# caojiezhang/CiaoSR

Hardware: AMD Instinct MI355X
Metric: HR Mpix/s (RDN-CiaoSR x4, LocalImplicitSR forward_test) (higher is better)
Workload: dtype f32; 1 GPU; C3: RDN-CiaoSR (c64b16) x4, LR 1356x2040 -> 5424x8160 (DIV2K-shaped 2K LR), tiled inference: 117 tiles of 192x192 (overlap 32), random-init weights, fp32; scale=4, tiles=117, parallelism=tile-shard x1

## Files before the change

ciaosr_amd/csrc/csa_attn_v4_f32.hip:

```cpp
#include "ops.h"

namespace ciaosr {

typedef float f32x16 __attribute__((ext_vector_type(16)));
typedef int i32x4 __attribute__((ext_vector_type(4)));

constexpr int AV_KW = 10;
constexpr int AV_SW = 2 * AV_KW;
constexpr int AV_RS = AV_SW + 3;
constexpr int AV_C = 64;
constexpr int AV_NCOL = 4 * AV_KW;
constexpr int AV_BT = AV_NCOL * AV_C;
constexpr int AV_KP = AV_NCOL / 2;
constexpr int AV_SA = 14;
constexpr int AV_SB = 8;
constexpr int AV_PF = 4;
static_assert(AV_SA % 2 == 0 && AV_SB % 2 == 0 && AV_PF % 2 == 0 && AV_KP % 2 == 0 && AV_SA > 0 && AV_SA + AV_PF <= AV_KP && AV_SB > 0 &&
              AV_SB < AV_KP, "k-pair groups; half 1 is not read before the barrier that completes it");

template <int QW>
struct AvCfg {
    static constexpr int NP = 256;
    static constexpr int NT = 2 * NP + 64 * (QW / 48);
    static constexpr int TR = NP / AV_RS;
    static constexpr int NI = (QW + 3 + TR - 1) / TR;
    static constexpr int NRB = TR * NI;
    static constexpr int PST = 4 * NRB * AV_RS;
    static constexpr int AT = AV_NCOL * QW;
    static constexpr size_t LDS = (size_t)(2 * AV_BT + PST + 2 * AT) * sizeof(float);
};
static_assert(AvCfg<192>::LDS <= 163840 && AvCfg<96>::LDS <= 163840, "LDS");
static_assert(AvCfg<192>::NP >= 192 + AV_KW - 1 && AvCfg<96>::NP >= 96 + AV_KW - 1, "one thread per diagonal");
static_assert(AvCfg<192>::NRB >= 192 + 3 && AvCfg<96>::NRB >= 96 + 3, "staged rows");
static_assert(2 * AV_BT >= (AV_KW - 1) * AV_RS && 2 * AvCfg<96>::AT >= (AV_KW + 2) * AV_RS + AV_RS, "diagonal read guard");

#ifdef CIAOSR_PROBE
__device__ unsigned long long g_avprobe[1024 * 48];
#define AVPROBE_T() __builtin_readcyclecounter()
#else
#define AVPROBE_T() 0ull
#endif

struct CsaAv4P {
    const float* S; const float2* st; const float* Pc; float* part;
    int Hp, Wp, Hh, Wh, Lld, nseg, nch, n_wg;
    int ys, oy0, noy;
    unsigned s_bytes, pc_bytes;
};

__device__ __forceinline__ void av_phase_barrier() {
    asm volatile("" ::: "memory");
    __builtin_amdgcn_s_barrier();
    asm volatile("" ::: "memory");
}

template <int QW>
__global__ __launch_bounds__(AvCfg<QW>::NT) void csa_attn_v4_kernel(CsaAv4P p) {
    using Cfg = AvCfg<QW>;
    constexpr int NP = Cfg::NP, TR = Cfg::TR, NI = Cfg::NI, NRB = Cfg::NRB;
    constexpr int NB = (AV_BT / 4 + NP - 1) / NP;
    extern __shared__ __attribute__((aligned(16))) float avs[];
    float* Bt = avs;
    float* Pst = avs + 2 * AV_BT;
    float* At = Pst + Cfg::PST;

    const int bid = blockIdx.x;
    const int q8 = p.n_wg >> 3, r8 = p.n_wg & 7;
    const int xcd = bid & 7, slot0 = bid >> 3;
    const int lid = (xcd < r8 ? xcd * (q8 + 1) : r8 * (q8 + 1) + (xcd - r8) * q8) + slot0;
    const int oy = p.oy0 + lid % p.noy, rest = lid / p.noy;
    const int seg = rest % p.nseg, quarter = rest / p.nseg;
    const int x0 = seg * QW, nq = min(QW, p.Wp - x0);
    const int ngy = p.Hh + 3, gyb = quarter * ngy / 4, nr = (quarter + 1) * ngy / 4 - gyb;
    const int HWp = p.Hp * p.Wp;
    const int nsteps = nr * p.nch;

    const int t = threadIdx.x, lane = t & 63, w = __builtin_amdgcn_readfirstlane(t >> 6);
#ifdef CIAOSR_PROBE
    const bool stamp = QW == 192 && lane == 0 && (w & 3) == 0 && bid < 1024;
    unsigned long long pacc[10] = {0, 0, 0, 0, 0, 0, 0, 0, 0, 0};
    const unsigned long long pstart = AVPROBE_T();
#define AVPROBE_ADD(slot, t0) do { const unsigned long long now_ = AVPROBE_T(); pacc[slot] += now_ - (t0); (t0) = now_; } while (0)
#define AVPROBE_OUT(role) do { if (stamp) { for (int i_ = 0; i_ < 10; ++i_) g_avprobe[bid * 48 + 16 * (role) + i_] = pacc[i_];                \
        g_avprobe[bid * 48 + 16 * (role) + 14] = AVPROBE_T() - pstart; g_avprobe[bid * 48 + 16 * (role) + 15] = (unsigned long long)nsteps; } } while (0)
#else
#define AVPROBE_ADD(slot, t0) do { } while (0)
#define AVPROBE_OUT(role) do { } while (0)
#endif

    int trow = 0, ch = 0;
    int gy = gyb + oy % nr, gx0 = 0;
    auto next_step = [&]() __attribute__((always_inline)) {
        if (++ch == p.nch) { ch = 0; ++trow; }
        gy = gyb + (trow + oy) % nr; gx0 = ch * AV_SW;
    };

    if (w < NP / 64) {
        const __amdgpu_buffer_rsrc_t rs_s = __builtin_amdgcn_make_buffer_rsrc(const_cast<float*>(p.S), 0, p.s_bytes, 0x00020000);
        const bool stager = t < TR * AV_RS;
        const int sj = t % AV_RS, sr0 = t / AV_RS;
        float negm[4][NI];
#pragma unroll
        for (int dyi = 0; dyi < 4; ++dyi) {
            const int qy = oy + dyi - 2;
#pragma unroll
            for (int i = 0; i < NI; ++i) {
                const int qx = x0 + sr0 + TR * i - 2;
                float v = -__builtin_inff();
                if (stager && qy >= 0 && qy < p.Hp && qx >= 0 && qx < p.Wp) {
                    const float2 s2 = p.st[(size_t)qy * p.Wp + qx];
                    v = -(s2.x - __builtin_amdgcn_logf(s2.y));
                }
                negm[dyi][i] = v;
            }
        }
        const int s_thread = sr0 * p.Lld + sj;
        const int s_istep = TR * p.Lld;
        float ra[4][NI];
        auto issue_logits = [&](auto dy0_c) __attribute__((always_inline)) {
            constexpr int DY0 = decltype(dy0_c)::value;
#pragma unroll
            for (int dyi = DY0; dyi < DY0 + 2; ++dyi) {
                const int dy = dyi - 2;
                const int base = ((oy + dy - p.ys) * p.Wp + x0 - 2) * p.Lld + (gy - 1 + dy) * p.Wh + gx0 - 3 + s_thread;
#pragma unroll
                for (int i = 0; i < NI; ++i)
                    ra[dyi][i] = __int_as_float(__builtin_amdgcn_raw_buffer_load_b32(rs_s, (base + i * s_istep) * 4, 0, 0));
            }
        };
        auto stage = [&](auto edge_c) __attribute__((always_inline)) {
            constexpr bool EDGE = decltype(edge_c)::value;
            constexpr float kL2e = 1.4426950408889634f;
            const bool kx = (unsigned)(gx0 - 3 + sj) < (unsigned)p.Wh;
#pragma unroll
            for (int dyi = 0; dyi < 4; ++dyi) {
                const bool ok = kx && (unsigned)(gy - 3 + dyi) < (unsigned)p.Hh;
                float* dst = Pst + dyi * NRB * AV_RS + sr0 * AV_RS + sj;
#pragma unroll
                for (int i = 0; i < NI; ++i) {
                    float v = __builtin_amdgcn_exp2f(__builtin_fmaf(ra[dyi][i], kL2e, negm[dyi][i]));
                    if (EDGE) v = ok ? v : 0.f;
                    if (stager) dst[i * TR * AV_RS] = v;
                }
                __builtin_amdgcn_sched_barrier(0);
            }
        };
        issue_logits(std::integral_constant<int, 0>{});
        issue_logits(std::integral_constant<int, 2>{});
        [[maybe_unused]] unsigned long long pt0 = AVPROBE_T();
#pragma unroll 1
        for (int step = 0; step < nsteps; ++step) {
            const bool edge = gy < 3 || gy >= p.Hh || gx0 < 3 || gx0 + AV_SW - 1 >= p.Wh;
            if (edge) stage(std::true_type{});
            else stage(std::false_type{});
            AVPROBE_ADD(0, pt0);
            __syncthreads();
            AVPROBE_ADD(1, pt0);
            next_step();
            const bool more = step + 1 < nsteps;
            if (more) issue_logits(std::integral_constant<int, 0>{});
            AVPROBE_ADD(2, pt0);
            __syncthreads();
            AVPROBE_ADD(3, pt0);
            if (more) issue_logits(std::integral_constant<int, 2>{});
            AVPROBE_ADD(4, pt0);
            __syncthreads();
            AVPROBE_ADD(5, pt0);
        }
        AVPROBE_OUT(0);
        return;
    }

    if (w < 2 * NP / 64) {
        const int td = t - NP;
        const __amdgpu_buffer_rsrc_t rs_pc = __builtin_amdgcn_make_buffer_rsrc(const_cast<float*>(p.Pc), 0, p.pc_bytes, 0x00020000);
        int b_rel[NB], b_k[NB];
#pragma unroll
        for (int s = 0; s < NB; ++s) {
            const int idx = td + NP * s, kk = idx >> 4, c4 = idx & 15;
            const int blk = kk / AV_KW, k = kk - blk * AV_KW;
            const int pcb = blk == 0 ? 8 : blk == 1 ? 6 : blk == 2 ? 2 : 0;
            b_rel[s] = k * 9 * AV_C + pcb * AV_C + 4 * c4;
            b_k[s] = idx < AV_BT / 4 ? k : 0x40000000;
        }
        float4 rb[2][NB];
        auto issue_u = [&]() __attribute__((always_inline)) {
#pragma unroll
            for (int h = 0; h < 2; ++h) {
                const int brow = (gy * (p.Wh + 3) + gx0 + AV_KW * h) * 9 * AV_C;
#pragma unroll
                for (int s = 0; s < NB; ++s) {
                    const unsigned off = gx0 + AV_KW * h + b_k[s] < p.Wh + 3 ? (unsigned)(brow + b_rel[s]) * 4u : 0x80000000u;
                    const i32x4 v = __builtin_amdgcn_raw_buffer_load_b128(rs_pc, off, 0, 0);
                    rb[h][s] = make_float4(__int_as_float(v.x), __int_as_float(v.y), __int_as_float(v.z), __int_as_float(v.w));
                }
            }
        };
        const int c = td - (AV_KW - 1);
        const bool diag = td < QW + AV_KW - 1;
        const float* dsrc = Pst + c * AV_RS;
        float* adst0 = At + c;
        auto half = [&](auto h_c) __attribute__((always_inline)) {
            constexpr int H = decltype(h_c)::value;
#pragma unroll
            for (int s = 0; s < NB; ++s)
                if (NP * (s + 1) <= AV_BT / 4 || td + NP * s < AV_BT / 4)
                    *reinterpret_cast<float4*>(Bt + H * AV_BT + 4 * (td + NP * s)) = rb[H][s];
            if (diag) {
                float* adst = adst0 + H * Cfg::AT;
                float xa2[AV_KW], xb2[AV_KW], ya[AV_KW], yb[AV_KW];
#pragma unroll
                for (int dyi = 0; dyi < 4; ++dyi) {
                    float d[AV_KW + 3];
#pragma unroll
                    for (int j = 0; j < AV_KW + 3; ++j) d[j] = dsrc[dyi * NRB * AV_RS + AV_KW * H + j * (AV_RS + 1)];
#pragma unroll
                    for (int k = 0; k < AV_KW; ++k) {
                        const float pr = d[k + 1] + d[k + 2];
                        const float xa = pr + d[k + 3], xb = pr + d[k];
                        if (dyi == 0) { xa2[k] = xa; xb2[k] = xb; }
                        else if (dyi == 1) { ya[k] = xa; yb[k] = xb; }
                        else if (dyi == 2) {
                            ya[k] = ya[k] + xa; yb[k] = yb[k] + xb;
                            if ((unsigned)(c + k) < (unsigned)nq) {
                                adst[(2 * AV_KW + k) * QW + k] = ya[k] + xa2[k];
                                adst[(3 * AV_KW + k) * QW + k] = yb[k] + xb2[k];
                            }
                        } else if ((unsigned)(c + k) < (unsigned)nq) {
                            adst[(0 * AV_KW + k) * QW + k] = ya[k] + xa;
                            adst[(1 * AV_KW + k) * QW + k] = yb[k] + xb;
                        }
                    }
                }
            }
        };
        [[maybe_unused]] unsigned long long pt0 = AVPROBE_T();
#pragma unroll 1
        for (int step = 0; step < nsteps; ++step) {
            issue_u();
            __syncthreads();
            AVPROBE_ADD(0, pt0);
            half(std::integral_constant<int, 0>{});
            AVPROBE_ADD(1, pt0);
            __syncthreads();
            AVPROBE_ADD(2, pt0);
            half(std::integral_constant<int, 1>{});
            next_step();
            AVPROBE_ADD(3, pt0);
            __syncthreads();
            AVPROBE_ADD(4, pt0);
        }
        AVPROBE_OUT(1);
        return;
    }

    const int cw = w - 2 * NP / 64, wm = cw >> 1, wn = cw & 1, li = lane & 31, lh = lane >> 5;
    f32x16 acc[3];
#pragma unroll
    for (int mi = 0; mi < 3; ++mi)
#pragma unroll
        for (int r = 0; r < 16; ++r) acc[mi][r] = 0.f;
    const float* fa = At + lh * QW + wm * 96 + li;
    const float* fb = Bt + lh * AV_C + wn * 32 + li;
    [[maybe_unused]] unsigned long long ct0 = AVPROBE_T();
    auto mma_step = [&](auto nbar_c) __attribute__((always_inline)) {
        constexpr int NBAR = decltype(nbar_c)::value, NE = 2 * AV_KP;
        float a[NE][3], b[NE];
        auto ld = [&](int e) __attribute__((always_inline)) {
            const int h = e / AV_KP, kp = e - h * AV_KP;
            b[e] = fb[h * AV_BT + 2 * kp * AV_C];
#pragma unroll
            for (int mi = 0; mi < 3; ++mi) a[e][mi] = fa[h * Cfg::AT + 2 * kp * QW + mi * 32];
        };
#pragma unroll
        for (int e = 0; e < AV_PF; ++e) ld(e);
#pragma unroll
        for (int e = 0; e < NE; e += 2) {
            if (e + AV_PF < NE) { ld(e + AV_PF); ld(e + AV_PF + 1); }
            __builtin_amdgcn_sched_barrier(0);
#pragma unroll
            for (int u = 0; u < 2; ++u)
#pragma unroll
                for (int mi = 0; mi < 3; ++mi)
                    acc[mi] = __builtin_amdgcn_mfma_f32_32x32x2f32(a[e + u][mi], b[e + u], acc[mi], 0, 0, 0);
            __builtin_amdgcn_sched_barrier(0);
            if (NBAR >= 1 && e + 2 == AV_SA) {
                AVPROBE_ADD(0, ct0);
                av_phase_barrier();
                AVPROBE_ADD(1, ct0);
            }
            if (NBAR >= 2 && e + 2 == AV_KP + AV_SB) {
                AVPROBE_ADD(2, ct0);
                av_phase_barrier();
                AVPROBE_ADD(3, ct0);
            }
        }
    };
    if (nsteps > 0) {
        av_phase_barrier();
        __syncthreads();
    }
    ct0 = AVPROBE_T();
#pragma unroll 1
    for (int step = 0; step + 1 < nsteps; ++step) {
        mma_step(std::integral_constant<int, 2>{});
        AVPROBE_ADD(4, ct0);
        __syncthreads();
        AVPROBE_ADD(5, ct0);
    }
    if (nsteps > 0) mma_step(std::integral_constant<int, 1>{});
    AVPROBE_OUT(2);

    float* dst = p.part + ((size_t)quarter * HWp + (size_t)oy * p.Wp + x0) * AV_C + wn * 32 + li;
#pragma unroll
    for (int mi = 0; mi < 3; ++mi)
#pragma unroll
        for (int r = 0; r < 16; ++r) {
            const int row = wm * 96 + mi * 32 + (r & 3) + 8 * (r >> 2) + 4 * lh;
            if (row < nq) dst[(size_t)row * AV_C] = acc[mi][r];
        }
}
#undef AVPROBE_ADD
#undef AVPROBE_OUT


__device__ __forceinline__ int av_subset(int d) { return d == -2 ? 0 : (d == 1 ? 2 : 1); }

__global__ void csa_gather_vedge_kernel(const float* __restrict__ Pc, int Hh, int Wh, int C, float* __restrict__ Ve) {
    const int c4n = C >> 2;
    const long n = (long)Hh * Wh * 9 * c4n;
    const int We = Wh + 3;
    for (long idx = blockIdx.x * (long)blockDim.x + threadIdx.x; idx < n; idx += (long)gridDim.x * blockDim.x) {
        const int c4 = (int)(idx % c4n);
        const long t = idx / c4n;
        const int blk = (int)(t % 9);
        const int l = (int)(t / 9);
        const int ly = l / Wh, lx = l - ly * Wh;
        int dy, dx, r, sct;
        if (blk < 4) { dy = 0; dx = blk - 2; r = 0; sct = av_subset(dx); }
        else if (blk < 8) { dy = blk - 6; dx = 0; r = av_subset(dy); sct = 0; }
        else { dy = 0; dx = 0; r = 0; sct = 0; }
        const size_t src = ((size_t)(ly - dy + 1) * We + (lx - dx + 1)) * (9 * C) + (size_t)(3 * r + sct) * C + 4 * c4;
        reinterpret_cast<float4*>(Ve)[idx] = *reinterpret_cast<const float4*>(Pc + src);
    }
}

__global__ void csa_attn_v4_combine_kernel(const float* __restrict__ part, const float* __restrict__ Otop, const float* __restrict__ Oleft,
                                           const float* __restrict__ Otl, const float* __restrict__ bd, int H, int W, int Hp, int Wp,
                                           int C, float* __restrict__ out, int ld_out) {
    const int c4n = C >> 2;
    const long n = (long)H * W * c4n;
    const size_t qs = (size_t)Hp * Wp * C;
    for (long idx = blockIdx.x * (long)blockDim.x + threadIdx.x; idx < n; idx += (long)gridDim.x * blockDim.x) {
        const int c4 = (int)(idx % c4n);
        const long pix = idx / c4n;
        const int x = (int)(pix % W), y = (int)(pix / W);
        const size_t o = ((size_t)y * Wp + x) * C + 4 * c4;
        float4 acc = *reinterpret_cast<const float4*>(part + o);
#pragma unroll
        for (int q = 1; q < 4; ++q) {
            const float4 v = *reinterpret_cast<const float4*>(part + q * qs + o);
            acc.x += v.x; acc.y += v.y; acc.z += v.z; acc.w += v.w;
        }
        if (y == 0 || x == 0) {
            float4 e = make_float4(0.f, 0.f, 0.f, 0.f);
            if (y == 0)
                for (int dx = -2; dx <= 1; ++dx) {
                    if (x + dx < 0 || x + dx >= Wp) continue;
                    const float4 v = *reinterpret_cast<const float4*>(Otop + (size_t)(x + dx) * 4 * C + (size_t)(dx + 2) * C + 4 * c4);
                    e.x += v.x; e.y += v.y; e.z += v.z; e.w += v.w;
                }
            if (x == 0)
                for (int dy = -2; dy <= 1; ++dy) {
                    if (y + dy < 0 || y + dy >= Hp) continue;
                    const float4 v = *reinterpret_cast<const float4*>(Oleft + (size_t)(y + dy) * 4 * C + (size_t)(dy + 2) * C + 4 * c4);
                    e.x += v.x; e.y += v.y; e.z += v.z; e.w += v.w;
                }
            if (y == 0 && x == 0) {
                const float4 v = *reinterpret_cast<const float4*>(Otl + 4 * c4);
                e.x -= v.x; e.y -= v.y; e.z -= v.z; e.w -= v.w;
            }
            acc.x -= e.x; acc.y -= e.y; acc.z -= e.z; acc.w -= e.w;
        }
        const float4 b = *reinterpret_cast<const float4*>(bd + 4 * c4);
        acc.x = (b.x + acc.x) / 6.f; acc.y = (b.y + acc.y) / 6.f; acc.z = (b.z + acc.z) / 6.f; acc.w = (b.w + acc.w) / 6.f;
        *reinterpret_cast<float4*>(out + (size_t)pix * ld_out + 4 * c4) = acc;
    }
}

static inline int av_grid(long n) {
    long g = (n + 255) / 256;
    return (int)(g < 1 ? 1 : (g > 4096 ? 4096 : g));
}

bool csa_attn_v4_ok(int Hp, int Wp, int C, int Lld, int s_rows) {
    return C == AV_C && Hp >= 4 && Wp >= 4 && (Hp & 1) == 0 && (Wp & 1) == 0 && (Lld & 3) == 0 && s_rows >= 1 &&
           (size_t)s_rows * Wp * Lld * sizeof(float) < 0x80000000ull;
}

int csa_attn_v4_f32(const float* S, int Lld, const float* stats2, const float* Pc, float* part, int Hp, int Wp, int C, bool tile128,
                    int ys, int s_rows, int oy0, int oy1, hipStream_t s) {
    CIAOSR_CHECK_ARG(S && stats2 && Pc && part && csa_attn_v4_ok(Hp, Wp, C, Lld, s_rows) && aligned16(Pc) && aligned16(part));
    CIAOSR_CHECK_ARG(0 <= oy0 && oy0 < oy1 && oy1 <= Hp && ys >= 0 && ys + s_rows <= Hp && ys <= (oy0 > 2 ? oy0 - 2 : 0) &&
                     ys + s_rows >= (oy1 < Hp ? oy1 + 1 : Hp));
    CsaAv4P p;
    p.S = S; p.st = reinterpret_cast<const float2*>(stats2); p.Pc = Pc; p.part = part;
    p.Hp = Hp; p.Wp = Wp; p.Hh = Hp / 2; p.Wh = Wp / 2; p.Lld = Lld;
    const int qw = tile128 ? 96 : 192;
    p.nseg = ceil_div(Wp, qw);
    p.nch = ceil_div(p.Wh + 3, AV_SW);
    p.ys = ys; p.oy0 = oy0; p.noy = oy1 - oy0;
    p.n_wg = p.noy * p.nseg * 4;
    p.s_bytes = (unsigned)((size_t)s_rows * Wp * Lld * sizeof(float));
    p.pc_bytes = (unsigned)((size_t)(p.Hh + 3) * (p.Wh + 3) * 9 * C * sizeof(float));
    ProfScope prof("csa_attn_v", s);
    if (tile128) {
        CIAOSR_BIG_LDS(csa_attn_v4_kernel<96>, AvCfg<96>::LDS);
        hipLaunchKernelGGL(csa_attn_v4_kernel<96>, dim3(p.n_wg), dim3(AvCfg<96>::NT), AvCfg<96>::LDS, s, p);
    } else {
        CIAOSR_BIG_LDS(csa_attn_v4_kernel<192>, AvCfg<192>::LDS);
        hipLaunchKernelGGL(csa_attn_v4_kernel<192>, dim3(p.n_wg), dim3(AvCfg<192>::NT), AvCfg<192>::LDS, s, p);
    }
    return launch_status("csa_attn_v4_f32");
}

int csa_gather_vedge(const float* Pc, int Hh, int Wh, int C, float* Ve, hipStream_t s) {
    ProfScope prof("csa_gather_vedge", s);
    hipLaunchKernelGGL(csa_gather_vedge_kernel, dim3(av_grid((long)Hh * Wh * 9 * C / 4)), dim3(256), 0, s, Pc, Hh, Wh, C, Ve);
    return launch_status("csa_gather_vedge");
}

int csa_attn_v4_combine(const float* part, const float* Otop, const float* Oleft, const float* Otl, const float* bd, int H, int W, int Hp,
                        int Wp, int C, float* out, int ld_out, hipStream_t s) {
    ProfScope prof("csa_gather_out", s);
    hipLaunchKernelGGL(csa_attn_v4_combine_kernel, dim3(av_grid((long)H * W * C / 4)), dim3(256), 0, s, part, Otop, Oleft, Otl, bd, H, W,
                       Hp, Wp, C, out, ld_out);
    return launch_status("csa_attn_v4_combine");
}

}

#ifdef CIAOSR_PROBE
extern "C" int ciaosr_debug_probe_av4_read(unsigned long long* host, int n_words) {
    return hipMemcpyFromSymbol(host, HIP_SYMBOL(ciaosr::g_avprobe), (size_t)n_words * 8) == hipSuccess ? 0 : -1;
}
#endif
```

ciaosr_amd/csrc/csa_scores_f32.hip:

```cpp
#include "ops.h"

namespace ciaosr {

typedef float f32x16 __attribute__((ext_vector_type(16)));
typedef int i32x4 __attribute__((ext_vector_type(4)));

constexpr int BSH = 8, BSW = 16;
constexpr int BLH = 4, BLW = 16;
constexpr int BHW = BSW + 2;
constexpr int BPN = (BSH + 2) * BHW;
constexpr int BLN = (BLH + 2) * BHW;
constexpr int BDP = 109;
constexpr int BDB = BPN * BDP * 4;
constexpr size_t kBoxLds = 2 * (size_t)BDB;
constexpr unsigned kOobB = 0xFFFFFFF0u;

struct BoxP {
    const float* M; int ldm; unsigned m_bytes; int Hp, Wp;
    int y0, y1;
    const float* R; int ldr; unsigned r_bytes; int Hl, Wl;
    const float* nrm;
    float* S; int lds_; size_t s_floats;
    int pbx, lbx, n_lb, n_items;
};

__global__ void csa_key_norms_kernel(const float* __restrict__ R, int ldr, int Hl, int Wl, int Ch, float floor_, float alpha,
                                     float* __restrict__ nrm) {
    const int lane = threadIdx.x & 63;
    const long l = (long)blockIdx.x * 4 + (threadIdx.x >> 6);
    if (l >= (long)Hl * Wl) return;
    const int ly = (int)(l / Wl), lx = (int)(l - (long)ly * Wl);
    float ss = 0.f;
    for (int e = lane; e < 9 * Ch; e += 64) {
        const int tap = e / Ch, c = e - tap * Ch;
        const int y = ly + tap / 3 - 1, x = lx + tap % 3 - 1;
        if (y >= 0 && y < Hl && x >= 0 && x < Wl) {
            const float v = R[((size_t)y * Wl + x) * ldr + c];
            ss += v * v;
        }
    }
#pragma unroll
    for (int o = 32; o > 0; o >>= 1) ss += __shfl_xor(ss, o, 64);
    if (lane == 0) nrm[l] = alpha / fmaxf(sqrtf(ss), floor_);
}

__global__ __launch_bounds__(512) void csa_scores_box_f32_kernel(BoxP p) {
    extern __shared__ __attribute__((aligned(16))) float Dl[];
    const int t = threadIdx.x, lane = t & 63, wv = __builtin_amdgcn_readfirstlane(t >> 6), li = lane & 31, lh = lane >> 5;
    const int per = (p.n_items + (int)gridDim.x - 1) / (int)gridDim.x;
    const int i0 = (int)blockIdx.x * per, i1 = min(i0 + per, p.n_items);
    if (i0 >= i1) return;
    auto item_pb = [&](int it) -> int { return it / p.n_lb; };
    auto item_lb = [&](int it) -> int { return it - (it / p.n_lb) * p.n_lb; };

    if (wv < 4) {
        const __amdgpu_buffer_rsrc_t rs_m = __builtin_amdgcn_make_buffer_rsrc(const_cast<float*>(p.M), 0, p.m_bytes, 0x00020000);
        const __amdgpu_buffer_rsrc_t rs_r = __builtin_amdgcn_make_buffer_rsrc(const_cast<float*>(p.R), 0, p.r_bytes, 0x00020000);
        auto row_off = [&](int h, int hn, int y0, int x0, int Hh, int Ww, int ld) -> unsigned {
            const int hy = h / BHW, hx = h - hy * BHW;
            const int y = y0 - 1 + hy, x = x0 - 1 + hx;
            return (h < hn && y >= 0 && y < Hh && x >= 0 && x < Ww) ? (unsigned)(((size_t)y * Ww + x) * ld * 4) + (unsigned)lh * 16u : kOobB;
        };
        i32x4 fa[6][4];
        i32x4 fbc[4], fbn[4];
        auto load_a = [&](int pb) {
            const int py0 = p.y0 + (pb / p.pbx) * BSH, px0 = (pb % p.pbx) * BSW;
#pragma unroll
            for (int pt = 0; pt < 6; ++pt) {
                const unsigned mo = row_off(32 * pt + li, BPN, py0, px0, p.Hp, p.Wp, p.ldm);
#pragma unroll
                for (int j = 0; j < 4; ++j) fa[pt][j] = __builtin_amdgcn_raw_buffer_load_b128(rs_m, mo == kOobB ? (int)kOobB : (int)(mo + 32u * j), 0, 0);
            }
        };
        auto load_b = [&](int lb, i32x4 (&f)[4]) {
            const int ly0 = (lb / p.lbx) * BLH, lx0 = (lb % p.lbx) * BLW;
            const unsigned ro = row_off(32 * wv + li, BLN, ly0, lx0, p.Hl, p.Wl, p.ldr);
#pragma unroll
            for (int j = 0; j < 4; ++j) f[j] = __builtin_amdgcn_raw_buffer_load_b128(rs_r, ro == kOobB ? (int)kOobB : (int)(ro + 32u * j), 0, 0);
        };
        int cur_pb = item_pb(i0);
        load_a(cur_pb);
        load_b(item_lb(i0), fbc);
#pragma unroll 1
        for (int it = i0; it <= i1; ++it) {
            if (it < i1) {
                const int k = (it - i0) & 1;
                if (it + 1 < i1) load_b(item_lb(it + 1), fbn);
                float* D = Dl + k * (BDB / 4);
                const int lcol = 32 * wv + li;
#pragma unroll
                for (int pt = 0; pt < 6; ++pt) {
                    f32x16 acc;
#pragma unroll
                    for (int e = 0; e < 16; ++e) acc[e] = 0.f;
#pragma unroll
                    for (int j = 0; j < 4; ++j) {
                        const i32x4 a = fa[pt][j], b = fbc[j];
                        acc = __builtin_amdgcn_mfma_f32_32x32x2f32(__int_as_float(a.x), __int_as_float(b.x), acc, 0, 0, 0);
                        acc = __builtin_amdgcn_mfma_f32_32x32x2f32(__int_as_float(a.y), __int_as_float(b.y), acc, 0, 0, 0);
                        acc = __builtin_amdgcn_mfma_f32_32x32x2f32(__int_as_float(a.z), __int_as_float(b.z), acc, 0, 0, 0);
                        acc = __builtin_amdgcn_mfma_f32_32x32x2f32(__int_as_float(a.w), __int_as_float(b.w), acc, 0, 0, 0);
                    }
                    if (lcol < BLN) {
                        float* dcol = D + (4 * lh) * BDP + lcol;
#pragma unroll
                        for (int r = 0; r < 16; ++r) {
                            constexpr int kLast = BPN - 1;
                            const int rr = 32 * pt + (r & 3) + 8 * (r >> 2);
                            if (rr + 4 <= kLast) dcol[rr * BDP] = acc[r];
                            else if (rr <= kLast && lh == 0) dcol[rr * BDP] = acc[r];
                        }
                    }
                }
#pragma unroll
                for (int j = 0; j < 4; ++j) fbc[j] = fbn[j];
                if (it + 1 < i1 && item_pb(it + 1) != cur_pb) {
                    cur_pb = item_pb(it + 1);
                    load_a(cur_pb);
                }
            }
            __syncthreads();
        }
    } else {
        const int lyy = lane >> 4, lxx = lane & 15;
        int lcol9[9];
#pragma unroll
        for (int a = 0; a < 3; ++a)
#pragma unroll
            for (int b = 0; b < 3; ++b) lcol9[3 * a + b] = (lyy + a) * BHW + lxx + b;
        const int q0 = 32 * (wv - 4);
#pragma unroll 1
        for (int it = i0; it <= i1; ++it) {
            if (it > i0) {
                const int ci = it - 1, k = (ci - i0) & 1;
                const int pb = item_pb(ci), lb = item_lb(ci);
                const int py0 = p.y0 + (pb / p.pbx) * BSH, px0 = (pb % p.pbx) * BSW;
                const int ly = (lb / p.lbx) * BLH + lyy, lx = (lb % p.lbx) * BLW + lxx;
                const bool l_ok = ly < p.Hl && lx < p.Wl;
                const float sc = l_ok ? p.nrm[(size_t)ly * p.Wl + lx] : 0.f;
                const float* D = Dl + k * (BDB / 4) + (q0 >> 4) * BHW * BDP;
                const unsigned lane_off = l_ok ? (unsigned)((size_t)ly * p.Wl + lx) * 4u : kOobB;
                const int qy0 = py0 + (q0 >> 4);
                const size_t s_base = ((size_t)(qy0 - p.y0) * p.Wp + px0) * p.lds_;
                const size_t s_left = p.s_floats > s_base ? (p.s_floats - s_base) * 4 : 0;
                const size_t s_span = ((size_t)p.Wp + BSW) * p.lds_ * 4;
                const __amdgpu_buffer_rsrc_t rs_s =
                    __builtin_amdgcn_make_buffer_rsrc(p.S + s_base, 0, (unsigned)(s_left < s_span ? s_left : s_span), 0x00020000);
                const float* dk[9];
#pragma unroll
                for (int e = 0; e < 9; ++e) dk[e] = D + lcol9[e];
#pragma unroll
                for (int q = 0; q < 32; ++q) {
                    const int pyy = q >> 4, pxx = q & 15;
                    float s = dk[0][(pyy * BHW + pxx) * BDP];
#pragma unroll
                    for (int e = 1; e < 9; ++e) s += dk[e][((pyy + e / 3) * BHW + pxx + e % 3) * BDP];
                    const bool row_ok = qy0 + pyy < p.y1 && px0 + pxx < p.Wp;
                    const unsigned soff = (unsigned)(((size_t)pyy * p.Wp + pxx) * p.lds_ * 4);
                    __builtin_amdgcn_raw_buffer_store_b32(__float_as_int(s * sc), rs_s, (int)(row_ok ? lane_off : kOobB), (int)(row_ok ? soff : 0u), 0);
                }
            }
            __syncthreads();
        }
    }
}

bool csa_scores_box_ok(int Ch, int ldm, int ldr) { return Ch == 32 && (ldm & 3) == 0 && (ldr & 3) == 0; }

int csa_key_norms(const float* R, int ldr, int Hl, int Wl, int Ch, float alpha, float floor_, float* nrm, hipStream_t s) {
    CIAOSR_CHECK_ARG(R && nrm && csa_scores_box_ok(Ch, Ch, ldr));
    ProfScope prof("csa_key_norms", s);
    hipLaunchKernelGGL(csa_key_norms_kernel, dim3(ceil_div((long)Hl * Wl, 4)), dim3(256), 0, s, R, ldr, Hl, Wl, Ch, floor_, alpha, nrm);
    return launch_status("csa_key_norms");
}

int csa_scores_box_f32(const float* M, int ldm, int Hp, int Wp, const float* R, int ldr, int Hl, int Wl, int Ch, const float* nrm, float* S,
                       int ld_s, int y0, int y1, hipStream_t s) {
    CIAOSR_CHECK_ARG(M && R && nrm && S && csa_scores_box_ok(Ch, ldm, ldr) && aligned16(M) && aligned16(R) && 0 <= y0 && y0 < y1 && y1 <= Hp);
    const size_t mb = (size_t)Hp * Wp * ldm * 4, rb = (size_t)Hl * Wl * ldr * 4;
    const size_t s_floats = ((size_t)(y1 - y0) * Wp - 1) * ld_s + (size_t)Hl * Wl;
    CIAOSR_CHECK_ARG(mb < 0xFFFFFF00ull && rb < 0xFFFFFF00ull && ((size_t)Wp + BSW) * ld_s * 4 < 0xFFFFFF00ull);
    BoxP p;
    p.M = M; p.ldm = ldm; p.m_bytes = (unsigned)mb; p.Hp = Hp; p.Wp = Wp; p.y0 = y0; p.y1 = y1;
    p.R = R; p.ldr = ldr; p.r_bytes = (unsigned)rb; p.Hl = Hl; p.Wl = Wl;
    p.nrm = nrm; p.S = S; p.lds_ = ld_s; p.s_floats = s_floats;
    p.pbx = ceil_div(Wp, BSW); p.lbx = ceil_div(Wl, BLW);
    p.n_lb = ceil_div(Hl, BLH) * p.lbx;
    const long n_items = (long)ceil_div(y1 - y0, BSH) * p.pbx * p.n_lb;
    CIAOSR_CHECK_ARG(n_items < 0x7FFFFFFF);
    p.n_items = (int)n_items;
    CIAOSR_BIG_LDS(csa_scores_box_f32_kernel, kBoxLds);
    ProfScope prof("csa_scores", s);
    hipLaunchKernelGGL(csa_scores_box_f32_kernel, dim3(p.n_items < 256 ? p.n_items : 256), dim3(512), kBoxLds, s, p);
    return launch_status("csa_scores_box_f32");
}

}
```

Before: 12.15 Mpix/s.

## Pack attention and score-box LDS math into paired f32x2 ops with aligned blocks

Measured after the change: 12.21 Mpix/s (median of 6 runs). No clear change (+0.5%).

```diff
diff --git a/ciaosr_amd/csrc/csa_attn_v4_f32.hip b/ciaosr_amd/csrc/csa_attn_v4_f32.hip
--- a/ciaosr_amd/csrc/csa_attn_v4_f32.hip
+++ b/ciaosr_amd/csrc/csa_attn_v4_f32.hip
@@ -4,6 +4,8 @@
 
 typedef float f32x16 __attribute__((ext_vector_type(16)));
 typedef int i32x4 __attribute__((ext_vector_type(4)));
+typedef float f32x2 __attribute__((ext_vector_type(2)));
+typedef __attribute__((address_space(3))) const float* av_lds_cptr;
 
 constexpr int AV_KW = 10;
 constexpr int AV_SW = 2 * AV_KW;
@@ -25,13 +27,15 @@
     static constexpr int TR = NP / AV_RS;
     static constexpr int NI = (QW + 3 + TR - 1) / TR;
     static constexpr int NRB = TR * NI;
-    static constexpr int PST = 4 * NRB * AV_RS;
+    static constexpr int PB = (NRB * AV_RS + 63) / 64 * 64;
+    static constexpr int PST = 4 * PB;
     static constexpr int AT = AV_NCOL * QW;
     static constexpr size_t LDS = (size_t)(2 * AV_BT + PST + 2 * AT) * sizeof(float);
 };
 static_assert(AvCfg<192>::LDS <= 163840 && AvCfg<96>::LDS <= 163840, "LDS");
 static_assert(AvCfg<192>::NP >= 192 + AV_KW - 1 && AvCfg<96>::NP >= 96 + AV_KW - 1, "one thread per diagonal");
 static_assert(AvCfg<192>::NRB >= 192 + 3 && AvCfg<96>::NRB >= 96 + 3, "staged rows");
+static_assert(3 * AvCfg<192>::PB / 64 < 256 && AvCfg<192>::PB % 64 == 0 && AvCfg<96>::PB % 64 == 0, "ds_read2st64_b32 offsets of the four blocks");
 static_assert(2 * AV_BT >= (AV_KW - 1) * AV_RS && 2 * AvCfg<96>::AT >= (AV_KW + 2) * AV_RS + AV_RS, "diagonal read guard");
 
 #ifdef CIAOSR_PROBE
@@ -57,7 +61,7 @@
 template <int QW>
 __global__ __launch_bounds__(AvCfg<QW>::NT) void csa_attn_v4_kernel(CsaAv4P p) {
     using Cfg = AvCfg<QW>;
-    constexpr int NP = Cfg::NP, TR = Cfg::TR, NI = Cfg::NI, NRB = Cfg::NRB;
+    constexpr int NP = Cfg::NP, TR = Cfg::TR, NI = Cfg::NI, PB = Cfg::PB;
     constexpr int NB = (AV_BT / 4 + NP - 1) / NP;
     extern __shared__ __attribute__((aligned(16))) float avs[];
     float* Bt = avs;
@@ -99,7 +103,7 @@
         const __amdgpu_buffer_rsrc_t rs_s = __builtin_amdgcn_make_buffer_rsrc(const_cast<float*>(p.S), 0, p.s_bytes, 0x00020000);
         const bool stager = t < TR * AV_RS;
         const int sj = t % AV_RS, sr0 = t / AV_RS;
-        float negm[4][NI];
+        f32x2 negm[4][(NI + 1) / 2];
 #pragma unroll
         for (int dyi = 0; dyi < 4; ++dyi) {
             const int qy = oy + dyi - 2;
@@ -111,7 +115,7 @@
                     const float2 s2 = p.st[(size_t)qy * p.Wp + qx];
                     v = -(s2.x - __builtin_amdgcn_logf(s2.y));
                 }
-                negm[dyi][i] = v;
+                negm[dyi][i >> 1][i & 1] = v;
             }
         }
         const int s_thread = sr0 * p.Lld + sj;
@@ -135,12 +139,18 @@
 #pragma unroll
             for (int dyi = 0; dyi < 4; ++dyi) {
                 const bool ok = kx && (unsigned)(gy - 3 + dyi) < (unsigned)p.Hh;
-                float* dst = Pst + dyi * NRB * AV_RS + sr0 * AV_RS + sj;
-#pragma unroll
-                for (int i = 0; i < NI; ++i) {
-                    float v = __builtin_amdgcn_exp2f(__builtin_fmaf(ra[dyi][i], kL2e, negm[dyi][i]));
-                    if (EDGE) v = ok ? v : 0.f;
-                    if (stager) dst[i * TR * AV_RS] = v;
+                float* dst = Pst + dyi * PB + sr0 * AV_RS + sj;
+#pragma unroll
+                for (int i = 0; i < NI; i += 2) {
+                    f32x2 e;
+                    if (i + 1 < NI) e = __builtin_elementwise_fma(f32x2{ra[dyi][i], ra[dyi][i + 1]}, f32x2{kL2e, kL2e}, negm[dyi][i >> 1]);
+                    else e.x = __builtin_fmaf(ra[dyi][i], kL2e, negm[dyi][i >> 1].x);
+#pragma unroll
+                    for (int u = 0; u < 2 && i + u < NI; ++u) {
+                        float v = __builtin_amdgcn_exp2f(e[u]);
+                        if (EDGE) v = ok ? v : 0.f;
+                        if (stager) dst[(i + u) * TR * AV_RS] = v;
+                    }
                 }
                 __builtin_amdgcn_sched_barrier(0);
             }
@@ -198,7 +208,14 @@
         };
         const int c = td - (AV_KW - 1);
         const bool diag = td < QW + AV_KW - 1;
-        const float* dsrc = Pst + c * AV_RS;
+        av_lds_cptr dsrc[2][AV_KW + 3];
+#pragma unroll
+        for (int h = 0; h < 2; ++h)
+#pragma unroll
+            for (int j = 0; j < AV_KW + 3; ++j) {
+                dsrc[h][j] = (av_lds_cptr)(Pst + c * AV_RS + AV_KW * h + j * (AV_RS + 1));
+                asm volatile("" : "+v"(dsrc[h][j]));
+            }
         float* adst0 = At + c;
         auto half = [&](auto h_c) __attribute__((always_inline)) {
             constexpr int H = decltype(h_c)::value;
@@ -208,27 +225,25 @@
                     *reinterpret_cast<float4*>(Bt + H * AV_BT + 4 * (td + NP * s)) = rb[H][s];
             if (diag) {
                 float* adst = adst0 + H * Cfg::AT;
-                float xa2[AV_KW], xb2[AV_KW], ya[AV_KW], yb[AV_KW];
-#pragma unroll
-                for (int dyi = 0; dyi < 4; ++dyi) {
-                    float d[AV_KW + 3];
-#pragma unroll
-                    for (int j = 0; j < AV_KW + 3; ++j) d[j] = dsrc[dyi * NRB * AV_RS + AV_KW * H + j * (AV_RS + 1)];
+                f32x2 xa01[AV_KW], xb01[AV_KW];
+#pragma unroll
+                for (int pr_i = 0; pr_i < 2; ++pr_i) {
+                    f32x2 d[AV_KW + 3];
+#pragma unroll
+                    for (int j = 0; j < AV_KW + 3; ++j) d[j] = f32x2{dsrc[H][j][2 * pr_i * PB], dsrc[H][j][(2 * pr_i + 1) * PB]};
 #pragma unroll
                     for (int k = 0; k < AV_KW; ++k) {
-                        const float pr = d[k + 1] + d[k + 2];
-                        const float xa = pr + d[k + 3], xb = pr + d[k];
-                        if (dyi == 0) { xa2[k] = xa; xb2[k] = xb; }
-                        else if (dyi == 1) { ya[k] = xa; yb[k] = xb; }
-                        else if (dyi == 2) {
-                            ya[k] = ya[k] + xa; yb[k] = yb[k] + xb;
+                        const f32x2 pr = d[k + 1] + d[k + 2];
+                        const f32x2 xa = pr + d[k + 3], xb = pr + d[k];
+                        if (pr_i == 0) { xa01[k] = xa; xb01[k] = xb; }
+                        else {
+                            const float ya = xa01[k].y + xa.x, yb = xb01[k].y + xb.x;
                             if ((unsigned)(c + k) < (unsigned)nq) {
-                                adst[(2 * AV_KW + k) * QW + k] = ya[k] + xa2[k];
-                                adst[(3 * AV_KW + k) * QW + k] = yb[k] + xb2[k];
+                                adst[(2 * AV_KW + k) * QW + k] = ya + xa01[k].x;
+                                adst[(3 * AV_KW + k) * QW + k] = yb + xb01[k].x;
+                                adst[(0 * AV_KW + k) * QW + k] = ya + xa.y;
+                                adst[(1 * AV_KW + k) * QW + k] = yb + xb.y;
                             }
-                        } else if ((unsigned)(c + k) < (unsigned)nq) {
-                            adst[(0 * AV_KW + k) * QW + k] = ya[k] + xa;
-                            adst[(1 * AV_KW + k) * QW + k] = yb[k] + xb;
                         }
                     }
                 }
diff --git a/ciaosr_amd/csrc/csa_scores_f32.hip b/ciaosr_amd/csrc/csa_scores_f32.hip
--- a/ciaosr_amd/csrc/csa_scores_f32.hip
+++ b/ciaosr_amd/csrc/csa_scores_f32.hip
@@ -4,6 +4,7 @@
 
 typedef float f32x16 __attribute__((ext_vector_type(16)));
 typedef int i32x4 __attribute__((ext_vector_type(4)));
+typedef float f32x2 __attribute__((ext_vector_type(2)));
 
 constexpr int BSH = 8, BSW = 16;
 constexpr int BLH = 4, BLW = 16;
@@ -14,6 +15,13 @@
 constexpr int BDB = BPN * BDP * 4;
 constexpr size_t kBoxLds = 2 * (size_t)BDB;
 constexpr unsigned kOobB = 0xFFFFFFF0u;
+
+#ifdef CIAOSR_PROBE
+__device__ unsigned long long g_scprobe[256 * 16];
+#define SCPROBE_T() __builtin_readcyclecounter()
+#else
+#define SCPROBE_T() 0ull
+#endif
 
 struct BoxP {
     const float* M; int ldm; unsigned m_bytes; int Hp, Wp;
@@ -44,12 +52,29 @@
     if (lane == 0) nrm[l] = alpha / fmaxf(sqrtf(ss), floor_);
 }
 
-__global__ __launch_bounds__(512) void csa_scores_box_f32_kernel(BoxP p) {
+#ifdef __HIP_DEVICE_COMPILE__
+#define CSA_NO_LDS_MERGE __attribute__((target("no-load-store-opt")))
+#else
+#define CSA_NO_LDS_MERGE
+#endif
+
+__global__ __launch_bounds__(512) CSA_NO_LDS_MERGE void csa_scores_box_f32_kernel(BoxP p) {
     extern __shared__ __attribute__((aligned(16))) float Dl[];
     const int t = threadIdx.x, lane = t & 63, wv = __builtin_amdgcn_readfirstlane(t >> 6), li = lane & 31, lh = lane >> 5;
     const int per = (p.n_items + (int)gridDim.x - 1) / (int)gridDim.x;
     const int i0 = (int)blockIdx.x * per, i1 = min(i0 + per, p.n_items);
     if (i0 >= i1) return;
+#ifdef CIAOSR_PROBE
+    const bool stamp = lane == 0 && (wv & 3) == 0;
+    unsigned long long pacc[2] = {0, 0};
+    const unsigned long long pstart = SCPROBE_T();
+#define SCPROBE_ADD(slot, t0) do { const unsigned long long now_ = SCPROBE_T(); pacc[slot] += now_ - (t0); (t0) = now_; } while (0)
+#define SCPROBE_OUT(role) do { if (stamp) { unsigned long long* o_ = g_scprobe + blockIdx.x * 16 + 8 * (role); o_[0] = pacc[0]; o_[1] = pacc[1];   \
+        o_[2] = SCPROBE_T() - pstart; o_[3] = (unsigned long long)(i1 - i0); } } while (0)
+#else
+#define SCPROBE_ADD(slot, t0) do { } while (0)
+#define SCPROBE_OUT(role) do { } while (0)
+#endif
     auto item_pb = [&](int it) -> int { return it / p.n_lb; };
     auto item_lb = [&](int it) -> int { return it - (it / p.n_lb) * p.n_lb; };
 
@@ -81,6 +106,7 @@
         int cur_pb = item_pb(i0);
         load_a(cur_pb);
         load_b(item_lb(i0), fbc);
+        [[maybe_unused]] unsigned long long pt0 = SCPROBE_T();
 #pragma unroll 1
         for (int it = i0; it <= i1; ++it) {
             if (it < i1) {
@@ -119,8 +145,11 @@
                     load_a(cur_pb);
                 }
             }
+            SCPROBE_ADD(0, pt0);
             __syncthreads();
+            SCPROBE_ADD(1, pt0);
         }
+        SCPROBE_OUT(0);
     } else {
         const int lyy = lane >> 4, lxx = lane & 15;
         int lcol9[9];
@@ -129,6 +158,7 @@
 #pragma unroll
             for (int b = 0; b < 3; ++b) lcol9[3 * a + b] = (lyy + a) * BHW + lxx + b;
         const int q0 = 32 * (wv - 4);
+        [[maybe_unused]] unsigned long long pt0 = SCPROBE_T();
 #pragma unroll 1
         for (int it = i0; it <= i1; ++it) {
             if (it > i0) {
@@ -149,21 +179,44 @@
                 const float* dk[9];
 #pragma unroll
                 for (int e = 0; e < 9; ++e) dk[e] = D + lcol9[e];
-#pragma unroll
-                for (int q = 0; q < 32; ++q) {
-                    const int pyy = q >> 4, pxx = q & 15;
-                    float s = dk[0][(pyy * BHW + pxx) * BDP];
-#pragma unroll
-                    for (int e = 1; e < 9; ++e) s += dk[e][((pyy + e / 3) * BHW + pxx + e % 3) * BDP];
-                    const bool row_ok = qy0 + pyy < p.y1 && px0 + pxx < p.Wp;
-                    const unsigned soff = (unsigned)(((size_t)pyy * p.Wp + pxx) * p.lds_ * 4);
-                    __builtin_amdgcn_raw_buffer_store_b32(__float_as_int(s * sc), rs_s, (int)(row_ok ? lane_off : kOobB), (int)(row_ok ? soff : 0u), 0);
-                }
+                auto box = [&](auto interior_c) __attribute__((always_inline)) {
+                    constexpr bool INTERIOR = decltype(interior_c)::value;
+                    const f32x2 sc2 = {sc, sc};
+#pragma unroll
+                    for (int j = 0; j < 16; ++j) {
+                        const int pyy = j >> 3, pxx = 2 * (j & 7);
+                        f32x2 s = {dk[0][(pyy * BHW + pxx) * BDP], dk[0][(pyy * BHW + pxx + 1) * BDP]};
+#pragma unroll
+                        for (int e = 1; e < 9; ++e) {
+                            const int o = ((pyy + e / 3) * BHW + pxx + e % 3) * BDP;
+                            s += f32x2{dk[e][o], dk[e][o + BDP]};
+                        }
+                        s *= sc2;
+#pragma unroll
+                        for (int u = 0; u < 2; ++u) {
+                            const unsigned soff = (unsigned)(((size_t)pyy * p.Wp + pxx + u) * p.lds_ * 4);
+                            if (INTERIOR) {
+                                __builtin_amdgcn_raw_buffer_store_b32(__float_as_int(s[u]), rs_s, (int)lane_off, (int)soff, 0);
+                            } else {
+                                const bool row_ok = qy0 + pyy < p.y1 && px0 + pxx + u < p.Wp;
+                                __builtin_amdgcn_raw_buffer_store_b32(__float_as_int(s[u]), rs_s, (int)(row_ok ? lane_off : kOobB),
+                                                                      (int)(row_ok ? soff : 0u), 0);
+                            }
+                        }
+                    }
+                };
+                if (qy0 + 1 < p.y1 && px0 + BSW <= p.Wp) box(std::true_type{});
+                else box(std::false_type{});
             }
+            SCPROBE_ADD(0, pt0);
             __syncthreads();
+            SCPROBE_ADD(1, pt0);
         }
+        SCPROBE_OUT(1);
     }
 }
+#undef SCPROBE_ADD
+#undef SCPROBE_OUT
 
 bool csa_scores_box_ok(int Ch, int ldm, int ldr) { return Ch == 32 && (ldm & 3) == 0 && (ldr & 3) == 0; }
 
@@ -196,3 +249,9 @@
 }
 
 }
+
+#ifdef CIAOSR_PROBE
+extern "C" int ciaosr_debug_probe_scores_read(unsigned long long* host, int n_words) {
+    return hipMemcpyFromSymbol(host, HIP_SYMBOL(ciaosr::g_scprobe), (size_t)n_words * 8) == hipSuccess ? 0 : -1;
+}
+#endif
```
